# omerkurt-okt/buck-gnn

Measured on NVIDIA B200. Metric: graphs/sec, higher is better.
Workload: dtype f16

## Files before the change

### buckgnn_b200/csrc/aggregate.cuh

```cuda
#pragma once
#include <type_traits>
#include "common.cuh"

namespace bg {

constexpr int kHubSlices = 16;
constexpr int kAggWarpsPerBlock = 8;
#ifndef BG_AGG_THREADS16
#define BG_AGG_THREADS16 768
#endif
template <typename T> __host__ __device__ constexpr int agg_row_threads() { return sizeof(T) == 2 ? BG_AGG_THREADS16 : 512; }
template <typename T> __host__ __device__ constexpr int agg_fold_threads() { return agg_row_threads<T>(); }


template <int kAggr> BG_DEVINL float agg_init() { return kAggr == BG_AGGR_MAX ? -INFINITY : 0.f; }
template <int kAggr> BG_DEVINL float agg_op(float a, float b) {
  if constexpr (kAggr == BG_AGGR_MAX) return fmaxf(a, b); else return a + b;
}

template <typename T> struct RowFrag;

template <typename T> struct RowFrag16 {
  uint4 q[2];
  BG_DEVINL void load(const T* row, int lane) {
// ... 473 lines not shown
  if (threadIdx.x == 0) is_last = (atomicAdd(&ticket[hub], 1) == kHubSlices - 1);
  __syncthreads();
  if (!is_last) return;
  __threadfence();
  const float* hp = partial + (size_t)hub * kHubSlices * kHidden;
  T* orow = out + (size_t)(kCompact ? hub : r) * kHidden;
  for (int c = threadIdx.x; c < kHidden; c += blockDim.x) {
    float v = __ldcg(hp + c);
    for (int s = 1; s < kHubSlices; ++s) v = agg_op<kAggr>(v, __ldcg(hp + (size_t)s * kHidden + c));
    if constexpr (kAggr == BG_AGGR_MEAN) v = v / (float)max(deg, 1);
    if constexpr (sizeof(T) == 2) orow[c] = Pack16<T>::one(v); else orow[c] = v;
  }
  if (threadIdx.x == 0) ticket[hub] = 0;
}


template <typename T> struct Narrow {
  static constexpr int kCols = 128;
  static constexpr int kLanes = kCols * (int)sizeof(T) / 16;
  static constexpr int kVals = 16 / (int)sizeof(T);
  static constexpr int kRowsPerWarp = 32 / kLanes;
};

template <typename T, int kAggr>
BG_DEVINL void narrow_accumulate(float (&acc)[Narrow<T>::kVals], const uint4& q) {
  const uint32_t u[4] = {q.x, q.y, q.z, q.w};
  if constexpr (sizeof(T) == 2) {
#pragma unroll
    for (int i = 0; i < 4; ++i) {
      if constexpr (kAggr == BG_AGGR_MAX) {
        acc[2 * i] = fmaxf(acc[2 * i], Pack16<T>::lo(u[i]));
        acc[2 * i + 1] = fmaxf(acc[2 * i + 1], Pack16<T>::hi(u[i]));
      } else {
        Pack16<T>::add2(acc[2 * i], acc[2 * i + 1], u[i]);
      }
    }
  } else {
#pragma unroll
    for (int i = 0; i < 4; ++i) acc[i] = agg_op<kAggr>(acc[i], __uint_as_float(u[i]));
  }
}

template <typename T, int kAggr> BG_DEVINL uint4 narrow_neutral() {
  if constexpr (kAggr != BG_AGGR_MAX) return make_uint4(0u, 0u, 0u, 0u);
  else if constexpr (sizeof(T) == 4) return make_uint4(0xff800000u, 0xff800000u, 0xff800000u, 0xff800000u);
  else if constexpr (is_bf16<T>::value) return make_uint4(0xff80ff80u, 0xff80ff80u, 0xff80ff80u, 0xff80ff80u);
  else return make_uint4(0xfc00fc00u, 0xfc00fc00u, 0xfc00fc00u, 0xfc00fc00u);
}

template <typename T> BG_DEVINL uint4 narrow_pack(const float (&v)[Narrow<T>::kVals]) {
  uint4 o;
  if constexpr (sizeof(T) == 2) {
    o.x = Pack16<T>::pack(v[0], v[1]); o.y = Pack16<T>::pack(v[2], v[3]);
    o.z = Pack16<T>::pack(v[4], v[5]); o.w = Pack16<T>::pack(v[6], v[7]);
  } else {
    o.x = __float_as_uint(v[0]); o.y = __float_as_uint(v[1]); o.z = __float_as_uint(v[2]); o.w = __float_as_uint(v[3]);
  }
  return o;
}

template <typename T, int kAggr>
BG_DEVINL void narrow_gather(const T* __restrict__ x, const int32_t* __restrict__ col, int32_t beg, int32_t end,
                             int sl, uint32_t mask, float (&acc)[Narrow<T>::kVals]) {
  constexpr int kLanes = Narrow<T>::kLanes;
  const char* xb = reinterpret_cast<const char*>(x) + (size_t)sl * 16;
  constexpr size_t kRowBytes = 128 * sizeof(T);
  for (int32_t base = beg; base < end; base += kLanes) {
    const int32_t cnt = min(kLanes, end - base);
    const int32_t my = (sl < cnt) ? col[base + sl] : 0;
    int32_t j = 0;
    for (; j + 4 <= cnt; j += 4) {
      const uint4 q0 = ldg_v4(xb + (size_t)__shfl_sync(mask, my, j, kLanes) * kRowBytes);
      const uint4 q1 = ldg_v4(xb + (size_t)__shfl_sync(mask, my, j + 1, kLanes) * kRowBytes);
      const uint4 q2 = ldg_v4(xb + (size_t)__shfl_sync(mask, my, j + 2, kLanes) * kRowBytes);
      const uint4 q3 = ldg_v4(xb + (size_t)__shfl_sync(mask, my, j + 3, kLanes) * kRowBytes);
      narrow_accumulate<T, kAggr>(acc, q0); narrow_accumulate<T, kAggr>(acc, q1);
      narrow_accumulate<T, kAggr>(acc, q2); narrow_accumulate<T, kAggr>(acc, q3);
    }
    for (; j < cnt; ++j)
      narrow_accumulate<T, kAggr>(acc, ldg_v4(xb + (size_t)__shfl_sync(mask, my, j, kLanes) * kRowBytes));
  }
}

template <typename T, int kAggr>
__global__ void __launch_bounds__(1024, 1)
k_aggregate_rows128(const T* __restrict__ x, T* __restrict__ out, int64_t N,
                    const int32_t* __restrict__ rowptr, const int32_t* __restrict__ col) {
  using NW = Narrow<T>;
  constexpr int kLanes = NW::kLanes;
  constexpr uint32_t kFull = 0xffffffffu;
  const int lane = threadIdx.x & 31, warp = threadIdx.x >> 5;
  const int sub = lane / kLanes, sl = lane % kLanes;
  const int64_t band = (N + gridDim.x - 1) / gridDim.x;
  const int64_t r_beg = (int64_t)blockIdx.x * band;
  const int64_t r_end = min(N, r_beg + band);
  constexpr int kStride = 32 * NW::kRowsPerWarp;
  const char* xb = reinterpret_cast<const char*>(x) + (size_t)sl * 16;
  constexpr size_t kRowBytes = 128 * sizeof(T);
  auto offsets = [&](int64_t row, int32_t& b, int32_t& e) {
    b = 0; e = 0;
    if (row < r_end) { b = rowptr[row]; e = rowptr[row + 1]; }
  };
  int64_t r0 = r_beg + warp * NW::kRowsPerWarp;
  int32_t beg, end, nbeg, nend;
  offsets(r0 + sub, beg, end);
  int32_t my = (sl < end - beg) ? col[beg + sl] : 0;
  offsets(r0 + sub + kStride, nbeg, nend);
  for (; r0 < r_end; r0 += kStride) {
    const int64_t r = r0 + sub;
    const int32_t nmy = (sl < nend - nbeg) ? col[nbeg + sl] : 0;
    int32_t n2beg, n2end;
    offsets(r + 2 * kStride, n2beg, n2end);
    const int32_t deg = end - beg;
    const int32_t cnt = (deg <= kBigRowThreshold) ? min(deg, kLanes) : 0;
    int32_t wcnt = cnt;
    if constexpr (kLanes == 16) wcnt = max(wcnt, __shfl_xor_sync(kFull, cnt, 16));
    float acc[NW::kVals];
#pragma unroll
    for (int i = 0; i < NW::kVals; ++i) acc[i] = agg_init<kAggr>();
    for (int32_t base = 0; base < wcnt; base += 8) {
      auto round = [&](auto kN) {
        constexpr int n = decltype(kN)::value;
        uint4 q[n];
#pragma unroll
        for (int k = 0; k < n; ++k) {
          const int32_t nb = __shfl_sync(kFull, my, (base + k) & (kLanes - 1), kLanes);
          q[k] = narrow_neutral<T, kAggr>();
          if (base + k < cnt) q[k] = ldg_v4(xb + (size_t)nb * kRowBytes);
        }
#pragma unroll
        for (int k = 0; k < n; ++k) narrow_accumulate<T, kAggr>(acc, q[k]);
      };
      if (wcnt - base <= 5) round(std::integral_constant<int, 5>{});
      else round(std::integral_constant<int, 8>{});
    }
    if (deg <= kBigRowThreshold && r < r_end) {
      if (deg > kLanes) {
        const uint32_t mask = (kLanes == 32) ? kFull : (0xffffu << (16 * sub));
        narrow_gather<T, kAggr>(x, col, beg + kLanes, end, sl, mask, acc);
      }
      if constexpr (kAggr == BG_AGGR_MEAN) {
        const float d = (float)max(deg, 1);
        if constexpr (sizeof(T) == 4) {
#pragma unroll
          for (int i = 0; i < NW::kVals; ++i) acc[i] = acc[i] / d;
        } else {
          const float rd = 1.f / d;
#pragma unroll
          for (int i = 0; i < NW::kVals; ++i) acc[i] *= rd;
        }
      } else if constexpr (kAggr == BG_AGGR_MAX) {
        if (deg == 0) {
#pragma unroll
          for (int i = 0; i < NW::kVals; ++i) acc[i] = 0.f;
        }
      }
      stg_v4(reinterpret_cast<char*>(out) + (size_t)r * 128 * sizeof(T) + (size_t)sl * 16, narrow_pack<T>(acc));
    }
    beg = nbeg; end = nend; my = nmy; nbeg = n2beg; nend = n2end;
  }
}

template <typename T, int kAggr>
__global__ void __launch_bounds__(kAggWarpsPerBlock * 32)
k_aggregate_hubs128(const T* __restrict__ x, T* __restrict__ out,
                    const int32_t* __restrict__ rowptr, const int32_t* __restrict__ col,
                    const int32_t* __restrict__ big_rows, int32_t n_big,
                    float* __restrict__ partial, int32_t* __restrict__ ticket) {
  using NW = Narrow<T>;
  __shared__ float red[kAggWarpsPerBlock * NW::kRowsPerWarp][128];
  __shared__ int32_t is_last;
  const int lane = threadIdx.x & 31, warp = threadIdx.x >> 5;
  const int sub = lane / NW::kLanes, sl = lane % NW::kLanes;
  const uint32_t mask = (NW::kLanes == 32) ? 0xffffffffu : (0xffffu << (16 * sub));
  const int32_t hub = blockIdx.x / kHubSlices, slice = blockIdx.x % kHubSlices;
  if (hub >= n_big) return;
  const int32_t r = big_rows[hub];
  const int32_t beg = rowptr[r], deg = rowptr[r + 1] - beg;
  const int32_t s_beg = beg + (int32_t)((int64_t)deg * slice / kHubSlices);
  const int32_t s_end = beg + (int32_t)((int64_t)deg * (slice + 1) / kHubSlices);
  constexpr int kParts = kAggWarpsPerBlock * NW::kRowsPerWarp;
  const int part = warp * NW::kRowsPerWarp + sub;
  const int32_t s_len = s_end - s_beg;
  const int32_t w_beg = s_beg + (int32_t)((int64_t)s_len * part / kParts);
  const int32_t w_end = s_beg + (int32_t)((int64_t)s_len * (part + 1) / kParts);
  float acc[NW::kVals];
#pragma unroll
  for (int i = 0; i < NW::kVals; ++i) acc[i] = agg_init<kAggr>();
  narrow_gather<T, kAggr>(x, col, w_beg, w_end, sl, mask, acc);
#pragma unroll
  for (int i = 0; i < NW::kVals; ++i) red[part][sl * NW::kVals + i] = acc[i];
  __syncthreads();
  float* my_partial = partial + ((size_t)hub * kHubSlices + slice) * 128;
  for (int c = threadIdx.x; c < 128; c += blockDim.x) {
    float v = red[0][c];
#pragma unroll
    for (int w = 1; w < kParts; ++w) v = agg_op<kAggr>(v, red[w][c]);
    my_partial[c] = v;
  }
  __threadfence();
  __syncthreads();
  if (threadIdx.x == 0) is_last = (atomicAdd(&ticket[hub], 1) == kHubSlices - 1);
  __syncthreads();
  if (!is_last) return;
  __threadfence();
  const float* hp = partial + (size_t)hub * kHubSlices * 128;
  T* orow = out + (size_t)r * 128;
  for (int c = threadIdx.x; c < 128; c += blockDim.x) {
    float v = __ldcg(hp + c);
    for (int s2 = 1; s2 < kHubSlices; ++s2) v = agg_op<kAggr>(v, __ldcg(hp + (size_t)s2 * 128 + c));
    if constexpr (kAggr == BG_AGGR_MEAN) v = v / (float)max(deg, 1);
    if constexpr (sizeof(T) == 2) orow[c] = Pack16<T>::one(v); else orow[c] = v;
  }
  if (threadIdx.x == 0) ticket[hub] = 0;
}

}
```

### buckgnn_b200/csrc/capi.cu

```cuda
#include <cstdio>
#include <cstring>

#include "common.cuh"
#include "csr_build.cuh"
#include "aggregate.cuh"
#include "aggregate_window.cuh"
#include "encoder.cuh"
#include "gemm_tc.cuh"
#include "gemm128.cuh"
#include "pool_head.cuh"
#include "train.cuh"
#include "sag_pool.cuh"
#include "max_bwd.cuh"

namespace bg {

static thread_local char g_last_error[512] = "";

void set_last_cuda_error(cudaError_t e, const char* what, const char* file, int line) {
  snprintf(g_last_error, sizeof(g_last_error), "CUDA error %d (%s) at %s:%d: %s", (int)e,
           cudaGetErrorString(e), file, line, what);
}
static int fail(int code, const char* msg) {
  snprintf(g_last_error, sizeof(g_last_error), "%s", msg);
// ... 40 lines not shown
  int64_t stride = (int64_t)gridDim.x * blockDim.x;
  for (int64_t i = (int64_t)blockIdx.x * blockDim.x + threadIdx.x; i < n; i += stride)
    dst[i] = Pack16<T>::one(src[i]);
}
__global__ void k_split_tf32(const float* __restrict__ src, float* __restrict__ hi, float* __restrict__ lo, int64_t n) {
  int64_t stride = (int64_t)gridDim.x * blockDim.x;
  for (int64_t i = (int64_t)blockIdx.x * blockDim.x + threadIdx.x; i < n; i += stride) {
    const float v = src[i];
    const float h = __uint_as_float(__float_as_uint(v) & 0xffffe000u);
    if (hi) hi[i] = h;
    lo[i] = v - h;
  }
}

template <typename T>
__global__ void k_expand_rowptr(const int32_t* __restrict__ rowptr, int64_t n_rows, int32_t* __restrict__ row_of,
                                int32_t* __restrict__ iota, T* __restrict__ nonempty, int as_count) {
  const int lane = threadIdx.x & 31;
  const int64_t n_warps = ((int64_t)gridDim.x * blockDim.x) >> 5;
  for (int64_t r = (((int64_t)blockIdx.x * blockDim.x + threadIdx.x) >> 5); r < n_rows; r += n_warps) {
    const int32_t b = rowptr[r], e = rowptr[r + 1];
    if (row_of)
      for (int32_t i = b + lane; i < e; i += 32) { row_of[i] = (int32_t)r; iota[i] = i; }
    if (nonempty) {
      const int32_t deg = e - b;
      float v0 = 0.f;
      if (as_count) { if (lane < 3) v0 = (float)((deg >> (8 * lane)) & (lane == 2 ? 0x7fff : 0xff)); }
      else if (lane == 0 && deg > 0) v0 = 1.f;
      if constexpr (sizeof(T) == 2) { nonempty[r * 64 + lane] = Pack16<T>::one(v0); nonempty[r * 64 + 32 + lane] = Pack16<T>::one(0.f); }
      else { nonempty[r * 64 + lane] = v0; nonempty[r * 64 + 32 + lane] = 0.f; }
    }
  }
}

template <typename T>
__global__ void k_add(const T* __restrict__ a, const T* __restrict__ b, const T* __restrict__ c, T* __restrict__ out, int64_t n) {
  int64_t stride = (int64_t)gridDim.x * blockDim.x;
  for (int64_t i = (int64_t)blockIdx.x * blockDim.x + threadIdx.x; i < n; i += stride) {
    float v = (float)a[i] + (float)b[i];
    if (c) v += (float)c[i];
    if constexpr (sizeof(T) == 2) out[i] = Pack16<T>::one(v); else out[i] = v;
  }
}

__global__ void k_publish_words(const int32_t* __restrict__ src, volatile int32_t* __restrict__ dst_host, int n) {
  if ((int)threadIdx.x < n) dst_host[threadIdx.x] = src[threadIdx.x];
  __threadfence_system();
}


__global__ void __launch_bounds__(256)
k_expand_wire(const int32_t* __restrict__ wire_edges, int64_t E_wire, const int64_t* __restrict__ node_ptr,
              const int64_t* __restrict__ wire_ptr, const int64_t* __restrict__ full_ptr, int64_t G, int64_t E_full,
              int64_t* __restrict__ edge_index, int64_t* __restrict__ batch) {
  for (int64_t g = blockIdx.x; g < G; g += gridDim.x) {
    const int64_t n0 = node_ptr[g], n1 = node_ptr[g + 1];
    const int64_t w0 = wire_ptr[g], w1 = wire_ptr[g + 1];
    const int64_t f0 = full_ptr[g], f1 = full_ptr[g + 1];
    for (int64_t i = threadIdx.x; i < w1 - w0; i += blockDim.x) {
      edge_index[f0 + i] = (int64_t)wire_edges[w0 + i];
      edge_index[E_full + f0 + i] = (int64_t)wire_edges[E_wire + w0 + i];
    }
    const int64_t hub_pairs = ((f1 - f0) - (w1 - w0)) / 2;
    const int64_t s = n1 - 1, base = f0 + (w1 - w0);
    for (int64_t i = threadIdx.x; i < hub_pairs; i += blockDim.x) {
      edge_index[base + 2 * i] = s;              edge_index[E_full + base + 2 * i] = n0 + i;
      edge_index[base + 2 * i + 1] = n0 + i;     edge_index[E_full + base + 2 * i + 1] = s;
    }
    for (int64_t i = n0 + threadIdx.x; i < n1; i += blockDim.x) batch[i] = g;
  }
}

static inline int64_t min64(int64_t a, int64_t b) { return a < b ? a : b; }
static inline unsigned grid_for(int64_t n, int threads, int max_blocks) {
  int64_t b = ceil_div64(n > 0 ? n : 1, threads);
  return (unsigned)(b < max_blocks ? b : max_blocks);
}

struct HubRangeArgs { const int32_t* hub_lo; const int32_t* hub_of_row; int32_t max_degree; float* partial; };

template <typename T> static inline unsigned agg_grid(int64_t N) {
  return (unsigned)min64(ceil_div64(N, agg_row_threads<T>() / 32), (int64_t)agg_sm_count());
}
static inline int64_t hub_parts(int64_t band, int32_t max_degree) { return ceil_div64(max_degree > 0 ? max_degree : 1, band) + 1; }

template <typename T>
static int aggregate_dispatch(const T* x, T* out, int64_t N, const int32_t* rowptr, const int32_t* col,
                              const int32_t* big_rows, int32_t n_big, int aggr, float* partial, int32_t* ticket,
                              int width, const HubRangeArgs& hr, cudaStream_t stream) {
  if (width == 128) {
    const unsigned grid128 = (unsigned)min64(ceil_div64(N, 32), (int64_t)sm_count());
    const unsigned hub_grid128 = (unsigned)n_big * kHubSlices;
#define BG_AGG128_CASE(A)                                                                                        \
  case A:                                                                                                        \
    k_aggregate_rows128<T, A><<<grid128, 1024, 0, stream>>>(x, out, N, rowptr, col);                             \
    if (n_big > 0)                                                                                               \
      k_aggregate_hubs128<T, A><<<hub_grid128, kAggWarpsPerBlock * 32, 0, stream>>>(x, out, rowptr, col,         \
                                                                                    big_rows, n_big, partial, ticket); \
    break;
    switch (aggr) {
      BG_AGG128_CASE(BG_AGGR_MEAN)
      BG_AGG128_CASE(BG_AGGR_SUM)
      BG_AGG128_CASE(BG_AGGR_MAX)
      default: return fail(BG_ERR_INVALID, "bg_sage_aggregate: bad aggr");
    }
#undef BG_AGG128_CASE
    BG_LAUNCH_OK();
    return BG_OK;
  }
  const unsigned grid = agg_grid<T>(N);
  const int64_t band = ceil_div64(N, grid);
  if constexpr (sizeof(T) == 2) {
    static const bool use_window = [] { const char* e = getenv("BG_AGG_WINDOW"); return e && e[0] == '1'; }();
    if (use_window) {
      const bool fold = hr.hub_lo && n_big > 0 && aggr != BG_AGGR_MAX;
      const HubFold hf = fold ? HubFold{hr.hub_of_row, hr.hub_lo, hr.partial, (int32_t)hub_parts(band, hr.max_degree)}
                              : HubFold{nullptr, nullptr, nullptr, 0};
#define BG_AGGW_LAUNCH(A, F)                                                                                          \
  {                                                                                                                   \
    static bool set = false;                                                                                          \
    if (!set) { BG_CUDA_OK(cudaFuncSetAttribute(k_aggregate_window<T, A, F>, cudaFuncAttributeMaxDynamicSharedMemorySize, kWinSmemBytes)); set = true; } \
    k_aggregate_window<T, A, F><<<grid, kWinThreads, kWinSmemBytes, stream>>>(x, out, N, band, rowptr, col, hf);      \
  }
      if (fold) {
        if (aggr == BG_AGGR_MEAN) { BG_AGGW_LAUNCH(BG_AGGR_MEAN, true); k_hub_finalize<T, BG_AGGR_MEAN><<<(unsigned)n_big, 128, 0, stream>>>(out, N, band, rowptr, big_rows, hf); }
        else if (aggr == BG_AGGR_SUM) { BG_AGGW_LAUNCH(BG_AGGR_SUM, true); k_hub_finalize<T, BG_AGGR_SUM><<<(unsigned)n_big, 128, 0, stream>>>(out, N, band, rowptr, big_rows, hf); }
        else return fail(BG_ERR_INVALID, "bg_sage_aggregate: bad aggr");
      } else {
        const unsigned hub_grid_w = (unsigned)n_big * kHubSlices;
        if (aggr == BG_AGGR_MEAN) { BG_AGGW_LAUNCH(BG_AGGR_MEAN, false); if (n_big > 0) k_aggregate_hubs<T, BG_AGGR_MEAN><<<hub_grid_w, kAggWarpsPerBlock * 32, 0, stream>>>(x, out, rowptr, col, big_rows, n_big, partial, ticket); }
        else if (aggr == BG_AGGR_SUM) { BG_AGGW_LAUNCH(BG_AGGR_SUM, false); if (n_big > 0) k_aggregate_hubs<T, BG_AGGR_SUM><<<hub_grid_w, kAggWarpsPerBlock * 32, 0, stream>>>(x, out, rowptr, col, big_rows, n_big, partial, ticket); }
        else if (aggr == BG_AGGR_MAX) { BG_AGGW_LAUNCH(BG_AGGR_MAX, false); if (n_big > 0) k_aggregate_hubs<T, BG_AGGR_MAX><<<hub_grid_w, kAggWarpsPerBlock * 32, 0, stream>>>(x, out, rowptr, col, big_rows, n_big, partial, ticket); }
        else return fail(BG_ERR_INVALID, "bg_sage_aggregate: bad aggr");
      }
#undef BG_AGGW_LAUNCH
      BG_LAUNCH_OK();
      return BG_OK;
    }
  }
  if (hr.hub_lo && n_big > 0) {
    constexpr int kThreads = agg_fold_threads<T>();
    HubFold hf{hr.hub_of_row, hr.hub_lo, hr.partial, (int32_t)hub_parts(band, hr.max_degree)};
    constexpr int smem = agg_fold_smem<T>();
#define BG_AGGF_CASE(A)                                                                                              \
  case A: {                                                                                                          \
    static bool set = false;                                                                                         \
    if (!set) {                                                                                                      \
      BG_CUDA_OK(cudaFuncSetAttribute(k_aggregate_rows<T, A, true, kThreads>, cudaFuncAttributeMaxDynamicSharedMemorySize, smem)); \
       \
      BG_CUDA_OK(cudaFuncSetAttribute(k_aggregate_rows<T, A, true, kThreads>, cudaFuncAttributePreferredSharedMemoryCarveout, \
                                      (smem + 1024) * 100 / (228 * 1024) + 1));                                      \
      set = true;                                                                                                    \
    }                                                                                                                \
    k_aggregate_rows<T, A, true, kThreads><<<grid, kThreads, smem, stream>>>(x, out, N, band, rowptr, col, hf);      \
    k_hub_finalize<T, A><<<(unsigned)n_big, 128, 0, stream>>>(out, N, band, rowptr, big_rows, hf);                   \
  } break;
    switch (aggr) {
      BG_AGGF_CASE(BG_AGGR_MEAN)
      BG_AGGF_CASE(BG_AGGR_SUM)
      default: return fail(BG_ERR_UNSUPPORTED, "bg_sage_aggregate: range hubs fold into mean / sum aggregation only");
    }
#undef BG_AGGF_CASE
    BG_LAUNCH_OK();
    return BG_OK;
  }
  const unsigned hub_grid = (unsigned)n_big * kHubSlices;
  const HubFold none{nullptr, nullptr, nullptr, 0};
#define BG_AGG_CASE(A)                                                                                       \
  case A:                                                                                                    \
    k_aggregate_rows<T, A, false, agg_row_threads<T>()><<<grid, agg_row_threads<T>(), 0, stream>>>(x, out, N, band, rowptr, col, none); \
    if (n_big > 0)                                                                                           \
      k_aggregate_hubs<T, A><<<hub_grid, kAggWarpsPerBlock * 32, 0, stream>>>(x, out, rowptr, col, big_rows, \
                                                                              n_big, partial, ticket);      \
    break;
  switch (aggr) {
    BG_AGG_CASE(BG_AGGR_MEAN)
    BG_AGG_CASE(BG_AGGR_SUM)
    BG_AGG_CASE(BG_AGGR_MAX)
// ... 135 lines not shown
    BG_LAUNCH_OK();
    k_csr_sort_small<<<(unsigned)ceil_div64(N, 256), 256, 0, stream>>>(rowptr, N, other, perm, col, info);
    BG_LAUNCH_OK();
    static bool attr_set = false;
    const int sort_smem = kSortSmemElems * (int)sizeof(int32_t);
    if (!attr_set) {
      BG_CUDA_OK(cudaFuncSetAttribute(k_csr_sort_big, cudaFuncAttributeMaxDynamicSharedMemorySize, sort_smem));
      attr_set = true;
    }
    k_csr_sort_big<<<sms, 1024, sort_smem, stream>>>(rowptr, big_rows, info, max_big, other, N, perm, col, hub_lo, hub_of_row);
    BG_LAUNCH_OK();
  }
  return BG_OK;
}

int bg_batch_info(const int64_t* batch, int64_t N, int32_t* info, void* stream_) {
  cudaStream_t stream = static_cast<cudaStream_t>(stream_);
  if (!info || N < 0 || (N > 0 && !batch)) return fail(BG_ERR_INVALID, "bg_batch_info: bad argument");
  BG_CUDA_OK(cudaMemsetAsync(info, 0, sizeof(int32_t) * 2, stream));
  if (N == 0) return BG_OK;
  k_batch_info<<<grid_for(N, 256, sm_count() * 8), 256, 0, stream>>>(batch, N, info);
  BG_LAUNCH_OK();
  return BG_OK;
}

int bg_graph_ptr_build(const int64_t* batch, int64_t N, int64_t G, int32_t* graph_ptr, void* stream_) {
  cudaStream_t stream = static_cast<cudaStream_t>(stream_);
  if (!graph_ptr || N < 0 || G < 0 || (N > 0 && !batch)) return fail(BG_ERR_INVALID, "bg_graph_ptr_build: bad argument");
  k_graph_ptr<<<grid_for(N + 1, 256, sm_count() * 8), 256, 0, stream>>>(batch, N, G, graph_ptr);
  BG_LAUNCH_OK();
  return BG_OK;
}

int bg_publish_words(const int32_t* src, int32_t* dst_host_mapped, int32_t n, void* stream_) {
  cudaStream_t stream = static_cast<cudaStream_t>(stream_);
  if (!src || !dst_host_mapped || n <= 0 || n > 256) return fail(BG_ERR_INVALID, "bg_publish_words: bad argument");
  k_publish_words<<<1, 256, 0, stream>>>(src, dst_host_mapped, n);
  BG_LAUNCH_OK();
  return BG_OK;
}

int bg_encoder_front(const float* x, int64_t N, int32_t F, const float* w1, const float* b1,
                     const float* w2, const float* b2, const int32_t* row_gather, void* out, int out_dtype,
                     int32_t* nonfinite_flag, void* stream_) {
  cudaStream_t stream = static_cast<cudaStream_t>(stream_);
  if (N < 0 || F <= 0 || F > kEncMaxF) return fail(BG_ERR_UNSUPPORTED, "bg_encoder_front: need 0 < n_features <= 32");
  if (N == 0) return BG_OK;
  if (!x || !w1 || !b1 || !w2 || !b2 || !out || !aligned16(out)) return fail(BG_ERR_INVALID, "bg_encoder_front: bad pointer");
  const int smem = (int)sizeof(EncoderSmem);
  const unsigned grid = (unsigned)min64(ceil_div64(N, kEncRows), (int64_t)sm_count() * 3);
#define BG_ENC_CASE(T)                                                                                         \
  {                                                                                                            \
    static bool set = false;                                                                                   \
    if (!set) { BG_CUDA_OK(cudaFuncSetAttribute(k_encoder_front<T>, cudaFuncAttributeMaxDynamicSharedMemorySize, smem)); set = true; } \
    k_encoder_front<T><<<grid, kEncThreads, smem, stream>>>(x, N, F, w1, b1, w2, b2, row_gather, static_cast<T*>(out)); \
  }
#define BG_ENC_MMA_CASE(T)                                                                                     \
  {                                                                                                            \
    const int msmem = (int)sizeof(EncoderMmaSmem);                                                             \
    static bool set = false;                                                                                   \
    if (!set) { BG_CUDA_OK(cudaFuncSetAttribute(k_encoder_front_mma<T>, cudaFuncAttributeMaxDynamicSharedMemorySize, msmem)); set = true; } \
    const unsigned mgrid = (unsigned)min64(ceil_div64(N, 16 * kEncMmaWarps), (int64_t)sm_count() * 2);        \
    k_encoder_front_mma<T><<<mgrid, kEncMmaWarps * 32, msmem, stream>>>(x, N, F, w1, b1, w2, b2, row_gather, static_cast<T*>(out), nonfinite_flag); \
  }
  if (out_dtype == BG_BF16) BG_ENC_MMA_CASE(__nv_bfloat16)
  else if (out_dtype == BG_F16) BG_ENC_MMA_CASE(__half)
  else if (out_dtype == BG_F32) BG_ENC_CASE(float)
  else return fail(BG_ERR_INVALID, "bg_encoder_front: bad out_dtype");
#undef BG_ENC_MMA_CASE
#undef BG_ENC_CASE
  BG_LAUNCH_OK();
  return BG_OK;
}

static size_t generic_hub_bytes(int32_t n_big) {
  return (size_t)n_big * kHubSlices * kHidden * sizeof(float) + (size_t)n_big * sizeof(int32_t) + 256;
}
int bg_aggregate_workspace_bytes(int32_t n_big, size_t* bytes_host) {
  if (!bytes_host || n_big < 0) return fail(BG_ERR_INVALID, "bg_aggregate_workspace_bytes: bad argument");
  *bytes_host = generic_hub_bytes(n_big);
  return BG_OK;
}

static size_t hubfold_bytes(int64_t N, int dtype, int32_t n_big, int32_t max_degree) {
  const unsigned grid = dtype == BG_F32 ? agg_grid<float>(N) : agg_grid<__half>(N);
  const int64_t band = ceil_div64(N > 0 ? N : 1, grid);
  return (size_t)n_big * (size_t)hub_parts(band, max_degree) * kMaxStreamWarps * kHidden * sizeof(float) + 256;
}
int bg_hubfold_workspace_bytes(int64_t N, int dtype, int32_t n_big, int32_t max_degree, size_t* bytes_host) {
  if (!bytes_host || n_big < 0 || N < 0 || max_degree < 0) return fail(BG_ERR_INVALID, "bg_hubfold_workspace_bytes: bad argument");
  const size_t a = generic_hub_bytes(n_big), b = hubfold_bytes(N, dtype, n_big, max_degree);
  *bytes_host = a > b ? a : b;
  return BG_OK;
}

int bg_sage_aggregate(const void* x, void* out, int dtype, int64_t N, int32_t width, const int32_t* rowptr,
                      const int32_t* col, const int32_t* big_rows, int32_t n_big, int aggr,
                      const int32_t* hub_lo, const int32_t* hub_of_row, int32_t hub_max_degree,
                      void* workspace, size_t workspace_bytes, void* stream_) {
  cudaStream_t stream = static_cast<cudaStream_t>(stream_);
  if (N < 0 || n_big < 0) return fail(BG_ERR_INVALID, "bg_sage_aggregate: bad size");
  if (width != 512 && width != 128) return fail(BG_ERR_UNSUPPORTED, "bg_sage_aggregate: width must be 512 or 128");
  if (N == 0) return BG_OK;
  if (!x || !out || !rowptr || !aligned16(x) || !aligned16(out)) return fail(BG_ERR_INVALID, "bg_sage_aggregate: bad pointer");
  if ((hub_lo != nullptr) != (hub_of_row != nullptr)) return fail(BG_ERR_INVALID, "bg_sage_aggregate: hub_lo and hub_of_row go together");
  float* partial = nullptr;
  int32_t* ticket = nullptr;
  HubRangeArgs hr{nullptr, nullptr, 0, nullptr};
  if (n_big > 0) {
    const bool fold = hub_lo != nullptr && width == 512;
    size_t need = generic_hub_bytes(n_big);
    if (fold) { const size_t f = hubfold_bytes(N, dtype, n_big, hub_max_degree); if (f > need) need = f; }
    if (!workspace || workspace_bytes < need || !big_rows) return fail(BG_ERR_WORKSPACE, "bg_sage_aggregate: workspace too small");
    if (fold) {
      hr = HubRangeArgs{hub_lo, hub_of_row, hub_max_degree, static_cast<float*>(workspace)};
    } else {
      partial = static_cast<float*>(workspace);
      ticket = reinterpret_cast<int32_t*>(static_cast<char*>(workspace) + (size_t)n_big * kHubSlices * kHidden * sizeof(float));
      BG_CUDA_OK(cudaMemsetAsync(ticket, 0, sizeof(int32_t) * (size_t)n_big, stream));
    }
  }
  if (dtype == BG_BF16)
    return aggregate_dispatch(static_cast<const __nv_bfloat16*>(x), static_cast<__nv_bfloat16*>(out), N, rowptr, col,
                              big_rows, n_big, aggr, partial, ticket, width, hr, stream);
  if (dtype == BG_F16)
    return aggregate_dispatch(static_cast<const __half*>(x), static_cast<__half*>(out), N, rowptr, col,
                              big_rows, n_big, aggr, partial, ticket, width, hr, stream);
  if (dtype == BG_F32)
    return aggregate_dispatch(static_cast<const float*>(x), static_cast<float*>(out), N, rowptr, col, big_rows, n_big,
                              aggr, partial, ticket, width, hr, stream);
  return fail(BG_ERR_INVALID, "bg_sage_aggregate: bad dtype");
}

static inline int umma_format_of(int dtype) { return dtype == BG_F16 ? 0 : (dtype == BG_BF16 ? 1 : (dtype == BG_F32 ? 2 : -1)); }

static int gemm512_impl(const bg_gemm_segment* segs, int32_t n_seg, int64_t m, int a_dtype, int b_dtype,
                        const bg_epilogue* epi, const bg_fused_aggregate* fuse, void* out, int out_dtype, int64_t ldo,
                        int cta_group, void* stream_) {
  cudaStream_t stream = static_cast<cudaStream_t>(stream_);
  if (!segs || n_seg < 1 || n_seg > BG_MAX_GEMM_SEGMENTS) return fail(BG_ERR_INVALID, "bg_gemm512: bad segment count");
  if (m < 0 || m >= 0x7fffffffLL) return fail(BG_ERR_INVALID, "bg_gemm512: bad m");
  if (m == 0) return BG_OK;
  const int a_fmt = umma_format_of(a_dtype), b_fmt = umma_format_of(b_dtype);
  if (a_fmt < 0 || b_fmt < 0 || a_fmt != b_fmt)
    return fail(BG_ERR_INVALID, "bg_gemm512: a_dtype and b_dtype must be the same (bf16, f16 or f32)");
  if (umma_format_of(out_dtype) < 0) return fail(BG_ERR_INVALID, "bg_gemm512: bad out_dtype");
  if (cta_group != 2) return fail(BG_ERR_UNSUPPORTED, "bg_gemm512: only cta_group = 2 is built");
  const bool tf32 = a_fmt == 2;
  const int esz = tf32 ? 4 : 2, osz = out_dtype == BG_F32 ? 4 : 2;
  const int kblk = kStageKBytes / esz;
  if (!out || !aligned16(out) || (ldo * osz) % 16 != 0 || ldo < kHidden) return fail(BG_ERR_INVALID, "bg_gemm512: bad out/ldo");
  GemmParams p;
  memset(&p, 0, sizeof(p));
  for (int s = 0; s < n_seg; ++s) {
    const bg_gemm_segment& g = segs[s];
    const bool gathered = fuse != nullptr && s == 0;
    if ((!g.a && !gathered) || !g.b || g.k <= 0 || g.k % kblk != 0) return fail(BG_ERR_UNSUPPORTED, "bg_gemm512: k must be a positive multiple of 64 (16-bit) / 32 (tf32)");
    if ((!gathered && (!aligned16(g.a) || (g.lda * esz) % 16 != 0 || g.lda < g.k)) || !aligned16(g.b) || (g.ldb * esz) % 16 != 0 || g.ldb < g.k)
      return fail(BG_ERR_INVALID, "bg_gemm512: operand alignment / leading dimension");
    const int groups = g.b_groups > 1 ? g.b_groups : 1;
    if (groups != (segs[0].b_groups > 1 ? segs[0].b_groups : 1)) return fail(BG_ERR_INVALID, "bg_gemm512: segments disagree on b_groups");
    if (groups > 1 && m != (int64_t)groups * kHidden) return fail(BG_ERR_INVALID, "bg_gemm512: b_groups needs m == b_groups * 512");
    int rc = gathered ? BG_OK : make_operand_map(&p.seg[s].a, g.a, m, g.k, g.lda, (uint32_t)a_fmt);
    if (rc == BG_OK) rc = make_operand_map(&p.seg[s].b, g.b, (int64_t)groups * kHidden, g.k, g.ldb, (uint32_t)b_fmt);
    if (rc != BG_OK) return fail(rc, "bg_gemm512: cuTensorMapEncodeTiled failed");
    p.kblocks[s] = g.k / kblk;
  }
  p.n_seg = n_seg;
  p.b_group_tiles = segs[0].b_groups > 1 ? kHidden / (kTileM * cta_group) : 0;
  p.k_elems_per_block = kblk;
  p.a_fmt = (uint32_t)a_fmt; p.b_fmt = (uint32_t)b_fmt;
  p.n_tiles = (int32_t)ceil_div64(m, kTileM * cta_group);
  p.m = m;
  for (int i = 0; i < kHidden; ++i) { p.bias[i] = 0.f; p.scale[i] = 1.f; p.shift[i] = 0.f; }
  if (epi) {
    if (epi->residual && (!aligned16(epi->residual) || (epi->ldr * osz) % 16 != 0 || epi->ldr < kHidden))
      return fail(BG_ERR_INVALID, "bg_gemm512: bad residual/ldr");
    if (epi->bn_scale_host && !epi->bn_shift_host) return fail(BG_ERR_INVALID, "bg_gemm512: bn_scale without bn_shift");
    if (epi->bias_host) memcpy(p.bias, epi->bias_host, sizeof(float) * kHidden);
    if (epi->bn_scale_host) {
      memcpy(p.scale, epi->bn_scale_host, sizeof(float) * kHidden);
      memcpy(p.shift, epi->bn_shift_host, sizeof(float) * kHidden);
    }
    p.normalize = epi->normalize; p.relu = epi->relu;
    for (int k = 0; k < 2; ++k) {
      if (!epi->gather[k]) break;
      if (!epi->gather_idx[k] || !aligned16(epi->gather[k]) || (epi->gather_ld * osz) % 16 != 0 || epi->gather_ld < kHidden)
        return fail(BG_ERR_INVALID, "bg_gemm512: bad gather operand");
      p.gather[k] = epi->gather[k]; p.gidx[k] = epi->gather_idx[k];
      p.n_gather = k + 1;
    }
    p.gather_ld = epi->gather_ld;
    if (p.n_gather > 0 && (epi->normalize || epi->residual))
      return fail(BG_ERR_UNSUPPORTED, "bg_gemm512: gathered addends cannot be combined with normalize or residual");
    p.residual = epi->residual; p.ldr = epi->ldr;
// ... 977 lines not shown
```

### buckgnn_b200/engine.py

```python
from __future__ import annotations

import os
from dataclasses import dataclass
from typing import Dict, List, Optional, Tuple

import torch

from . import capi

_TORCH = {capi.BG_BF16: torch.bfloat16, capi.BG_F16: torch.float16, capi.BG_F32: torch.float32}
PRECISION_FORMATS = {
    "fp16": (capi.BG_F16, capi.BG_F16),
    "bf16": (capi.BG_BF16, capi.BG_BF16),
    "tf32": (capi.BG_F32, capi.BG_F32),
    "fp32": (capi.BG_F32, capi.BG_F32),
}
PRECISIONS = tuple(PRECISION_FORMATS)


def default_precision(aggr: str) -> str:
    return "fp16" if aggr in ("mean", "max") else "tf32"


def _stream() -> int:
# ... 160 lines not shown
    parts: Tuple[torch.Tensor, ...]
    code: int = capi.BG_F32


def pack_linear(weight: torch.Tensor, precision: str) -> LinearPack:
    w = weight.detach().to(torch.float32).contiguous()
    k = w.shape[1]
    s = _stream()
    code = PRECISION_FORMATS[precision][1]
    if code != capi.BG_F32:
        out = torch.empty(w.shape, dtype=_TORCH[code], device=w.device)
        capi.cast_f32(w.data_ptr(), out.data_ptr(), code, w.numel(), s)
        return LinearPack(k, (out,), code)
    if precision == "tf32":
        return LinearPack(k, (w.clone(),), code)
    hi, lo = torch.empty_like(w), torch.empty_like(w)
    capi.split_tf32(w.data_ptr(), hi.data_ptr(), lo.data_ptr(), w.numel(), s)
    return LinearPack(k, (hi, lo), code)


@dataclass
class SageLayerPack:
    lin_l: LinearPack
    lin_r: LinearPack
    bias: torch.Tensor
    bn_scale: Optional[torch.Tensor]
    bn_shift: Optional[torch.Tensor]


def fold_batchnorm(bn: torch.nn.BatchNorm1d) -> Tuple[torch.Tensor, torch.Tensor]:
    scale = (bn.weight.detach().float() / torch.sqrt(bn.running_var.detach().float() + bn.eps))
    shift = (bn.bias.detach().float() - bn.running_mean.detach().float() * scale)
    return scale.cpu().contiguous(), shift.cpu().contiguous()


def host_vector(t: torch.Tensor) -> torch.Tensor:
    return t.detach().float().cpu().contiguous()


class Activation:

    def __init__(self, n: int, width: int, precision: str, device):
        self.precision = precision
        self.code = PRECISION_FORMATS[precision][0]
        self.dtype = _TORCH[self.code]
        self.data = torch.empty((n, width), dtype=self.dtype, device=device)
        self.hi = self.lo = None
        if precision == "fp32":
            self.hi = self.data
            self.lo = torch.empty_like(self.data)

    def refresh_split(self):
        if self.precision == "fp32":
            capi.split_tf32(self.data.data_ptr(), None, self.lo.data_ptr(), self.data.numel(), _stream())


def _segments(act: Activation, w: LinearPack):
    k = w.k
    ld = act.data.shape[1]
    if act.precision != "fp32":
        return [(act.data.data_ptr(), ld, w.parts[0].data_ptr(), k, k)]
    w_hi, w_lo = w.parts
    return [(act.hi.data_ptr(), ld, w_hi.data_ptr(), k, k),
            (act.hi.data_ptr(), ld, w_lo.data_ptr(), k, k),
            (act.lo.data_ptr(), ld, w_hi.data_ptr(), k, k)]


def gemm512(segs, m: int, precision: str, out: Activation, *, cta_group: int = 2, **epi) -> None:
    a_code, b_code = PRECISION_FORMATS[precision]
    capi.gemm512(segs, m, a_code, b_code, out.data.data_ptr(), out.code, out.data.shape[1], _stream(),
                 cta_group=cta_group, **epi)
    out.refresh_split()


def gemm(segs, m: int, precision: str, out: Activation, *, cta_group: int = 2, **epi) -> None:
    if out.data.shape[1] != 128:
        return gemm512(segs, m, precision, out, cta_group=cta_group, **epi)
    a_code, b_code = PRECISION_FORMATS[precision]
    capi.gemm128(segs, m, a_code, b_code, out.data.data_ptr(), out.code, out.data.shape[1], _stream(),
                 cta_group=cta_group, **epi)
    out.refresh_split()


def aggregate(x: Activation, out: Activation, idx: GraphIndex, aggr: str, fold_hubs: bool = True) -> None:
    width = x.data.shape[1]
    ws_bytes = capi.aggregate_workspace_bytes(idx.n_big)
    hub = {}
    if fold_hubs and idx.hub_lo is not None and width == 512 and aggr != "max":
        fold_bytes = capi.hubfold_workspace_bytes(idx.n_nodes, x.code, idx.n_big, idx.hub_max_degree)
        if fold_bytes <= x.data.numel() * x.data.element_size() // 4 + (1 << 20):
            ws_bytes = fold_bytes
            hub = dict(hub_lo=idx.hub_lo.data_ptr(), hub_of_row=idx.hub_of_row.data_ptr(),
                       hub_max_degree=idx.hub_max_degree)
    ws = torch.empty(ws_bytes, dtype=torch.uint8, device=x.data.device)
    with TIMERS.span("aggregate" if width == 512 else "aggregate128"):
        capi.sage_aggregate(x.data.data_ptr(), out.data.data_ptr(), x.code, idx.n_nodes, idx.rowptr.data_ptr(),
                            idx.col.data_ptr(), idx.big_rows.data_ptr(), idx.n_big, capi.AGGR_CODES[aggr],
                            ws.data_ptr(), ws_bytes, _stream(), width=width, **hub)
    out.refresh_split()


def encoder_hidden(x: torch.Tensor, enc_w: Dict[str, torch.Tensor], precision: str,
                   row_gather: Optional[torch.Tensor] = None, nonfinite: Optional[torch.Tensor] = None) -> "Activation":
    f = x.shape[1]
    n = x.shape[0] if row_gather is None else row_gather.shape[0]
    h = Activation(n, 128, precision, x.device)
    with TIMERS.span("encoder_front"):
        capi.encoder_front(x.data_ptr(), n, f, enc_w["w1"].data_ptr(), enc_w["b1"].data_ptr(),
                           enc_w["w2"].data_ptr(), enc_w["b2"].data_ptr(), h.data.data_ptr(), h.code, _stream(),
                           row_gather=_p(row_gather), nonfinite=_p(nonfinite))
    h.refresh_split()
    return h


@dataclass
class FoldedLayer0Pack:
    wl3: LinearPack
    wr3: LinearPack
    wgate: LinearPack
    bias: torch.Tensor
    bn_scale: Optional[torch.Tensor]
    bn_shift: Optional[torch.Tensor]
    as_count: bool
    bias_all_gated: Optional[torch.Tensor] = None


def pack_folded_layer0(enc_last: torch.nn.Linear, conv, bn, aggr: str, precision: str, width: int = 512) -> FoldedLayer0Pack:
    dev = conv.lin_l.weight.device
    d64 = lambda t: t.detach().to(torch.float64).cpu()
    W3, b3 = d64(enc_last.weight), d64(enc_last.bias)
    W3 = torch.nn.functional.pad(W3, (0, 128 - W3.shape[1]))
    Wl, bl, Wr = d64(conv.lin_l.weight), d64(conv.lin_l.bias), d64(conv.lin_r.weight)
    lp = lambda w: pack_linear(w.to(torch.float32).to(dev), precision)
    gate = torch.cat([(Wl @ b3)[:, None], torch.zeros(width, 63, dtype=torch.float64)], 1)
    if aggr in ("sum", "add"):
        gate[:, 1] = gate[:, 0] * 256.0
        gate[:, 2] = gate[:, 0] * 65536.0
    scale, shift = fold_batchnorm(bn) if bn is not None else (None, None)
    return FoldedLayer0Pack(lp(Wl @ W3), lp(Wr @ W3), lp(gate), (Wr @ b3 + bl).to(torch.float32).contiguous(),
                            scale, shift, aggr in ("sum", "add"),
                            bias_all_gated=(Wr @ b3 + bl + Wl @ b3).to(torch.float32).contiguous())


def sage_layer0_folded(h: "Activation", out: "Activation", idx: GraphIndex, w: FoldedLayer0Pack, *, aggr: str,
                       normalize: bool, relu: bool, cta_group: int = 2) -> None:
    n = idx.n_nodes
    mh = Activation(n, 128, h.precision, h.data.device)
    aggregate(h, mh, idx, aggr)
    segs = _segments(mh, w.wl3) + _segments(h, w.wr3)
    bias = w.bias
    if not w.as_count and not idx.has_empty_rows:
        bias = w.bias_all_gated
    else:
        ind = Activation(n, 64, h.precision, h.data.device)
        capi.expand_rowptr(idx.rowptr.data_ptr(), n, idx.n_edges, None, None, ind.data.data_ptr(), ind.code, _stream(),
                           as_count=w.as_count)
        ind.refresh_split()
        segs = segs + _segments(ind, w.wgate)[:2]
    with TIMERS.span("sage_update0"):
        gemm(segs, n, h.precision, out, cta_group=cta_group, bias=bias.data_ptr(), bn_scale=_p(w.bn_scale),
             bn_shift=_p(w.bn_shift), normalize=normalize, relu=relu)


def encoder_forward(x: torch.Tensor, enc_w: Dict[str, torch.Tensor], w3: LinearPack, precision: str,
                    out: Activation, cta_group: int, row_gather: Optional[torch.Tensor] = None,
                    nonfinite: Optional[torch.Tensor] = None) -> None:
    h = encoder_hidden(x, enc_w, precision, row_gather, nonfinite)
    n = h.data.shape[0]
    with TIMERS.span("encoder_gemm"):
        gemm(_segments(h, w3), n, precision, out, cta_group=cta_group, bias=enc_w["b3_host"].data_ptr())

# ... 333 lines not shown
```

Baseline: 29740.

## Fold hub rows into width-128 aggregation via streaming TMA warp

Extends the hub-folding scheme to the 128-wide aggregation kernel. One warp per block streams contiguous chunks of x into a shared-memory ring with bulk async copies and accumulates per-hub partial sums, while the remaining warps do the normal gather. A small finalize kernel then combines the partials and writes the hub rows. This replaces the separate scattered hub gather kernel. In exchange it gives up one gather warp, adds dynamic shared memory and a progress-based spin throttle, and needs more workspace.

```diff
diff --git a/buckgnn_b200/csrc/aggregate.cuh b/buckgnn_b200/csrc/aggregate.cuh
--- a/buckgnn_b200/csrc/aggregate.cuh
+++ b/buckgnn_b200/csrc/aggregate.cuh
@@ -579,21 +579,139 @@
   }
 }
 
-template <typename T, int kAggr>
+template <typename T> struct StreamGeom128 {
+  static constexpr int kWarps = 1;
+  static constexpr int kChunk = sizeof(T) == 2 ? 64 : 16;
+  static constexpr int kRing = sizeof(T) == 2 ? 3 : 6;
+  static_assert(kChunk % (4 * Narrow<T>::kRowsPerWarp) == 0 && kChunk <= 64 && kWarps <= kMaxStreamWarps, "stream geometry");
+};
+template <typename T> constexpr int agg128_fold_smem() {
+  return 1024 + StreamGeom128<T>::kWarps * StreamGeom128<T>::kRing * StreamGeom128<T>::kChunk * 128 * (int)sizeof(T);
+}
+
+template <typename T, int kAggr, bool kFold = false>
 __global__ void __launch_bounds__(1024, 1)
 k_aggregate_rows128(const T* __restrict__ x, T* __restrict__ out, int64_t N,
-                    const int32_t* __restrict__ rowptr, const int32_t* __restrict__ col) {
+                    const int32_t* __restrict__ rowptr, const int32_t* __restrict__ col, const HubFold hf) {
   using NW = Narrow<T>;
+  using SG = StreamGeom128<T>;
   constexpr int kLanes = NW::kLanes;
   constexpr uint32_t kFull = 0xffffffffu;
+  constexpr int kStream = kFold ? SG::kWarps : 0;
+  constexpr int kGatherWarps = 32 - kStream;
   const int lane = threadIdx.x & 31, warp = threadIdx.x >> 5;
   const int sub = lane / kLanes, sl = lane % kLanes;
   const int64_t band = (N + gridDim.x - 1) / gridDim.x;
   const int64_t r_beg = (int64_t)blockIdx.x * band;
   const int64_t r_end = min(N, r_beg + band);
-  constexpr int kStride = 32 * NW::kRowsPerWarp;
+  constexpr int kStride = kGatherWarps * NW::kRowsPerWarp;
+  constexpr size_t kRowBytes = 128 * sizeof(T);
+  extern __shared__ __align__(128) unsigned char agg_smem[];
+  volatile int32_t* progress = reinterpret_cast<volatile int32_t*>(agg_smem);
+  if constexpr (kFold) {
+    constexpr int kChunk = SG::kChunk, kRing = SG::kRing, kLead = kStride + kStreamLead;
+    constexpr uint32_t kBufBytes = kChunk * (uint32_t)kRowBytes;
+    constexpr int kIdRegs = (kChunk + 31) / 32;
+    const uint32_t bars = smem_u32(agg_smem) + 64;
+    unsigned char* bufs = agg_smem + 1024;
+    if (threadIdx.x == 0) {
+      *progress = 0;
+      for (int i = 0; i < kStream * kRing; ++i) mbar_init(bars + 8u * i, 1);
+      fence_mbar_init();
+    }
+    __syncthreads();
+    if (warp >= kGatherWarps) {
+      const int sw = warp - kGatherWarps;
+      float acc[NW::kVals];
+#pragma unroll
+      for (int i = 0; i < NW::kVals; ++i) acc[i] = 0.f;
+      int32_t cur_h = -1;
+      auto flush = [&]() {
+        if (cur_h >= 0) {
+          if constexpr (NW::kRowsPerWarp == 2) {
+#pragma unroll
+            for (int i = 0; i < NW::kVals; ++i) acc[i] += __shfl_xor_sync(kFull, acc[i], 16);
+          }
+          const int64_t slot = (int64_t)cur_h * hf.parts + ((int64_t)blockIdx.x - hf.hub_lo[cur_h] / band);
+          if (sub == 0) {
+            float4* dst = reinterpret_cast<float4*>(hf.partial + (slot * kStream + sw) * 128 + sl * NW::kVals);
+#pragma unroll
+            for (int j = 0; j < NW::kVals / 4; ++j) dst[j] = make_float4(acc[4 * j], acc[4 * j + 1], acc[4 * j + 2], acc[4 * j + 3]);
+          }
+        }
+#pragma unroll
+        for (int i = 0; i < NW::kVals; ++i) acc[i] = 0.f;
+      };
+      const int64_t n_rows = r_end - r_beg;
+      const int64_t n_chunks = (n_rows + kChunk - 1) / kChunk;
+      const uint32_t my_bars = bars + 8u * (uint32_t)(sw * kRing);
+      unsigned char* my_bufs = bufs + (size_t)sw * kRing * kBufBytes;
+      auto issue = [&](int64_t c, int slot) {
+        const int64_t row0 = r_beg + c * kChunk;
+        const uint32_t bytes = (uint32_t)min((int64_t)kChunk, r_end - row0) * (uint32_t)kRowBytes;
+        while ((c * kChunk) > (int64_t)*progress + kLead) __nanosleep(256);
+        mbar_arrive_expect_tx(my_bars + 8u * slot, bytes);
+        asm volatile("cp.async.bulk.shared::cluster.global.mbarrier::complete_tx::bytes [%0], [%1], %2, [%3];"
+                     ::"r"(smem_u32(my_bufs + (size_t)slot * kBufBytes)), "l"(x + (size_t)row0 * 128), "r"(bytes),
+                       "r"(my_bars + 8u * slot) : "memory");
+      };
+      if (lane == 0)
+        for (int k = 0; k < kRing; ++k)
+          if (sw + (int64_t)k * kStream < n_chunks) issue(sw + (int64_t)k * kStream, k);
+      struct Ids { int32_t h[kIdRegs]; };
+      auto hub_ids = [&](int64_t c) -> Ids {
+        Ids v;
+#pragma unroll
+        for (int j = 0; j < kIdRegs; ++j) {
+          const int k = 32 * j + lane;
+          const int64_t row = r_beg + c * kChunk + k;
+          v.h[j] = (c < n_chunks && k < kChunk && row < r_end) ? hf.hub_of_row[row] : -1;
+        }
+        return v;
+      };
+      Ids h_cur = hub_ids(sw), h_nxt = hub_ids(sw + kStream);
+      int64_t it = 0;
+      for (int64_t c = sw; c < n_chunks; c += kStream, ++it) {
+        const int slot = (int)(it % kRing);
+        const int64_t row0 = r_beg + c * kChunk;
+        const int rows = (int)min((int64_t)kChunk, r_end - row0);
+        const Ids h_nxt2 = hub_ids(c + 2 * (int64_t)kStream);
+        const Ids hmine = h_cur;
+        h_cur = h_nxt; h_nxt = h_nxt2;
+        mbar_wait(my_bars + 8u * slot, (uint32_t)(it / kRing) & 1u, 78u);
+        const uint4* buf = reinterpret_cast<const uint4*>(my_bufs + (size_t)slot * kBufBytes);
+        bool same = true;
+#pragma unroll
+        for (int j = 0; j < kIdRegs; ++j) same = same && (32 * j + lane >= kChunk || hmine.h[j] == cur_h);
+        const bool uniform = rows == kChunk && __all_sync(kFull, same) && cur_h >= 0;
+        if (uniform) {
+#pragma unroll
+          for (int k0 = 0; k0 < kChunk; k0 += 4 * NW::kRowsPerWarp) {
+            uint4 q[4];
+#pragma unroll
+            for (int k = 0; k < 4; ++k) q[k] = buf[(size_t)(k0 + k * NW::kRowsPerWarp) * kLanes + lane];
+#pragma unroll
+            for (int k = 0; k < 4; ++k) narrow_accumulate<T, BG_AGGR_SUM>(acc, q[k]);
+          }
+        } else {
+          for (int k = 0; k < rows; ++k) {
+            int32_t src = hmine.h[0];
+            if constexpr (kIdRegs > 1) { if (k >= 32) src = hmine.h[kIdRegs - 1]; }
+            static_assert(kIdRegs <= 2, "hub ids of a chunk");
+            const int32_t h = __shfl_sync(kFull, src, k & 31);
+            if (h != cur_h) { flush(); cur_h = h; }
+            if (h >= 0 && (k % NW::kRowsPerWarp) == sub) narrow_accumulate<T, BG_AGGR_SUM>(acc, buf[(size_t)k * kLanes + sl]);
+          }
+        }
+        __syncwarp();
+        const int64_t nc = c + (int64_t)kRing * kStream;
+        if (lane == 0 && nc < n_chunks) issue(nc, slot);
+      }
+      flush();
+      return;
+    }
+  }
   const char* xb = reinterpret_cast<const char*>(x) + (size_t)sl * 16;
-  constexpr size_t kRowBytes = 128 * sizeof(T);
   auto offsets = [&](int64_t row, int32_t& b, int32_t& e) {
     b = 0; e = 0;
     if (row < r_end) { b = rowptr[row]; e = rowptr[row + 1]; }
@@ -604,6 +722,9 @@
   int32_t my = (sl < end - beg) ? col[beg + sl] : 0;
   offsets(r0 + sub + kStride, nbeg, nend);
   for (; r0 < r_end; r0 += kStride) {
+    if constexpr (kFold) {
+      if (warp == 0 && lane == 0) *progress = (int32_t)(r0 - r_beg);
+    }
     const int64_t r = r0 + sub;
     const int32_t nmy = (sl < nend - nbeg) ? col[nbeg + sl] : 0;
     int32_t n2beg, n2end;
@@ -656,6 +777,35 @@
     }
     beg = nbeg; end = nend; my = nmy; nbeg = n2beg; nend = n2end;
   }
+  if constexpr (kFold) {
+    if (warp == 0 && lane == 0) *progress = 0x7fffffff - 2 * (kStride + kStreamLead);
+  }
+}
+
+template <typename T, int kAggr>
+__global__ void __launch_bounds__(128)
+k_hub_finalize128(T* __restrict__ out, int64_t N, int64_t band, const int32_t* __restrict__ rowptr,
+                  const int32_t* __restrict__ big_rows, const HubFold hf) {
+  constexpr int kStream = StreamGeom128<T>::kWarps, kStreamChunk = StreamGeom128<T>::kChunk;
+  const int32_t b = blockIdx.x;
+  const int c = threadIdx.x;
+  const int32_t r = big_rows[b];
+  const int64_t deg = rowptr[r + 1] - rowptr[r];
+  const int64_t lo = hf.hub_lo[b], hi = lo + deg;
+  const int64_t c0 = lo / band, c1 = (hi - 1) / band;
+  float acc = 0.f;
+  for (int64_t cb = c0; cb <= c1; ++cb) {
+    const int64_t a = max(lo, cb * band), e = min(min(hi, (cb + 1) * band), N);
+    const float* src = hf.partial + (((int64_t)b * hf.parts + (cb - c0)) * kStream) * 128 + c;
+    const int64_t qa = (a - cb * band) / kStreamChunk, qe = (e - 1 - cb * band) / kStreamChunk;
+#pragma unroll
+    for (int w = 0; w < kStream; ++w) {
+      const int64_t q0 = qa + (((w - qa) % kStream) + kStream) % kStream;
+      if (q0 <= qe) acc += __ldcg(src + (int64_t)w * 128);
+    }
+  }
+  if constexpr (kAggr == BG_AGGR_MEAN) acc = acc / (float)max(deg, (int64_t)1);
+  if constexpr (sizeof(T) == 2) out[(size_t)r * 128 + c] = Pack16<T>::one(acc); else out[(size_t)r * 128 + c] = acc;
 }
 
 template <typename T, int kAggr>
diff --git a/buckgnn_b200/csrc/capi.cu b/buckgnn_b200/csrc/capi.cu
--- a/buckgnn_b200/csrc/capi.cu
+++ b/buckgnn_b200/csrc/capi.cu
@@ -146,6 +146,7 @@
 template <typename T> static inline unsigned agg_grid(int64_t N) {
   return (unsigned)min64(ceil_div64(N, agg_row_threads<T>() / 32), (int64_t)agg_sm_count());
 }
+static inline unsigned agg128_grid(int64_t N) { return (unsigned)min64(ceil_div64(N, 32), (int64_t)sm_count()); }
 static inline int64_t hub_parts(int64_t band, int32_t max_degree) { return ceil_div64(max_degree > 0 ? max_degree : 1, band) + 1; }
 
 template <typename T>
@@ -153,11 +154,37 @@
                               const int32_t* big_rows, int32_t n_big, int aggr, float* partial, int32_t* ticket,
                               int width, const HubRangeArgs& hr, cudaStream_t stream) {
   if (width == 128) {
-    const unsigned grid128 = (unsigned)min64(ceil_div64(N, 32), (int64_t)sm_count());
+    const unsigned grid128 = agg128_grid(N);
+    if (hr.hub_lo && n_big > 0) {
+      const int64_t band = ceil_div64(N, grid128);
+      const HubFold hf{hr.hub_of_row, hr.hub_lo, hr.partial, (int32_t)hub_parts(band, hr.max_degree)};
+      constexpr int smem = agg128_fold_smem<T>();
+#define BG_AGG128F_CASE(A)                                                                                           \
+  case A: {                                                                                                          \
+    static bool set = false;                                                                                         \
+    if (!set) {                                                                                                      \
+      BG_CUDA_OK(cudaFuncSetAttribute(k_aggregate_rows128<T, A, true>, cudaFuncAttributeMaxDynamicSharedMemorySize, smem)); \
+      BG_CUDA_OK(cudaFuncSetAttribute(k_aggregate_rows128<T, A, true>, cudaFuncAttributePreferredSharedMemoryCarveout, \
+                                      (smem + 1024) * 100 / (228 * 1024) + 1));                                      \
+      set = true;                                                                                                    \
+    }                                                                                                                \
+    k_aggregate_rows128<T, A, true><<<grid128, 1024, smem, stream>>>(x, out, N, rowptr, col, hf);                    \
+    k_hub_finalize128<T, A><<<(unsigned)n_big, 128, 0, stream>>>(out, N, band, rowptr, big_rows, hf);                \
+  } break;
+      switch (aggr) {
+        BG_AGG128F_CASE(BG_AGGR_MEAN)
+        BG_AGG128F_CASE(BG_AGGR_SUM)
+        default: return fail(BG_ERR_UNSUPPORTED, "bg_sage_aggregate: range hubs fold into mean / sum aggregation only");
+      }
+#undef BG_AGG128F_CASE
+      BG_LAUNCH_OK();
+      return BG_OK;
+    }
     const unsigned hub_grid128 = (unsigned)n_big * kHubSlices;
+    const HubFold none{nullptr, nullptr, nullptr, 0};
 #define BG_AGG128_CASE(A)                                                                                        \
   case A:                                                                                                        \
-    k_aggregate_rows128<T, A><<<grid128, 1024, 0, stream>>>(x, out, N, rowptr, col);                             \
+    k_aggregate_rows128<T, A><<<grid128, 1024, 0, stream>>>(x, out, N, rowptr, col, none);                       \
     if (n_big > 0)                                                                                               \
       k_aggregate_hubs128<T, A><<<hub_grid128, kAggWarpsPerBlock * 32, 0, stream>>>(x, out, rowptr, col,         \
                                                                                     big_rows, n_big, partial, ticket); \
@@ -459,15 +486,20 @@
   return BG_OK;
 }
 
-static size_t hubfold_bytes(int64_t N, int dtype, int32_t n_big, int32_t max_degree) {
-  const unsigned grid = dtype == BG_F32 ? agg_grid<float>(N) : agg_grid<__half>(N);
-  const int64_t band = ceil_div64(N > 0 ? N : 1, grid);
-  return (size_t)n_big * (size_t)hub_parts(band, max_degree) * kMaxStreamWarps * kHidden * sizeof(float) + 256;
+static size_t hubfold_bytes(int64_t N, int dtype, int width, int32_t n_big, int32_t max_degree) {
+  const int64_t n = N > 0 ? N : 1;
+  const unsigned grid = width == 128 ? agg128_grid(n) : dtype == BG_F32 ? agg_grid<float>(n) : agg_grid<__half>(n);
+  const int64_t band = ceil_div64(n, grid);
+  return (size_t)n_big * (size_t)hub_parts(band, max_degree) * kMaxStreamWarps * width * sizeof(float) + 256;
 }
 int bg_hubfold_workspace_bytes(int64_t N, int dtype, int32_t n_big, int32_t max_degree, size_t* bytes_host) {
   if (!bytes_host || n_big < 0 || N < 0 || max_degree < 0) return fail(BG_ERR_INVALID, "bg_hubfold_workspace_bytes: bad argument");
-  const size_t a = generic_hub_bytes(n_big), b = hubfold_bytes(N, dtype, n_big, max_degree);
-  *bytes_host = a > b ? a : b;
+  size_t bytes = generic_hub_bytes(n_big);
+  for (const int width : {512, 128}) {
+    const size_t f = hubfold_bytes(N, dtype, width, n_big, max_degree);
+    if (f > bytes) bytes = f;
+  }
+  *bytes_host = bytes;
   return BG_OK;
 }
 
@@ -485,9 +517,9 @@
   int32_t* ticket = nullptr;
   HubRangeArgs hr{nullptr, nullptr, 0, nullptr};
   if (n_big > 0) {
-    const bool fold = hub_lo != nullptr && width == 512;
+    const bool fold = hub_lo != nullptr;
     size_t need = generic_hub_bytes(n_big);
-    if (fold) { const size_t f = hubfold_bytes(N, dtype, n_big, hub_max_degree); if (f > need) need = f; }
+    if (fold) { const size_t f = hubfold_bytes(N, dtype, width, n_big, hub_max_degree); if (f > need) need = f; }
     if (!workspace || workspace_bytes < need || !big_rows) return fail(BG_ERR_WORKSPACE, "bg_sage_aggregate: workspace too small");
     if (fold) {
       hr = HubRangeArgs{hub_lo, hub_of_row, hub_max_degree, static_cast<float*>(workspace)};
diff --git a/buckgnn_b200/engine.py b/buckgnn_b200/engine.py
--- a/buckgnn_b200/engine.py
+++ b/buckgnn_b200/engine.py
@@ -266,11 +266,16 @@
     out.refresh_split()
 
 
+FOLD_HUBS128 = True
+
+
 def aggregate(x: Activation, out: Activation, idx: GraphIndex, aggr: str, fold_hubs: bool = True) -> None:
     width = x.data.shape[1]
     ws_bytes = capi.aggregate_workspace_bytes(idx.n_big)
     hub = {}
-    if fold_hubs and idx.hub_lo is not None and width == 512 and aggr != "max":
+    if width == 128 and not FOLD_HUBS128:
+        fold_hubs = False
+    if fold_hubs and idx.hub_lo is not None and aggr != "max":
         fold_bytes = capi.hubfold_workspace_bytes(idx.n_nodes, x.code, idx.n_big, idx.hub_max_degree)
         if fold_bytes <= x.data.numel() * x.data.element_size() // 4 + (1 << 20):
             ws_bytes = fold_bytes
```

Measured after the change: 30070, median of 6. +1.1%, better.
